# kakaoenterprise/JORLDY

Hardware: AMD Instinct MI355X
Metric: env_steps_per_s (PPO CartPole sync, W=8 workers/GPU, T=128) (higher is better)
Workload: dtype f32

## Files before the change

jorldy_amd/csrc/jh_mlp.hip:

```cpp
#include "jh_ppo_mb.h"
#include "jh_netcore.h"
#include "jh_ppo_finish.h"

typedef float f32x4 __attribute__((ext_vector_type(4)));

namespace {
constexpr int kNormBlocks = 256;
constexpr int kNormSlots = kNormBlocks + 256;
constexpr int kMaxHeadOutputs = 40;
}

constexpr int kL1Rows = 16;
__global__ void __launch_bounds__(256) jh_mlp_l1_kernel(int B, int S, int H, const float* __restrict__ x,
                                                        const int64_t* __restrict__ idx, const float* __restrict__ W1,
                                                        const float* __restrict__ b1, float* __restrict__ h1) {
  __shared__ __attribute__((aligned(16))) float sx[kL1Rows][16];
  const int jb = (H + 255) / 256;
  const int rb = blockIdx.x / jb, j = (blockIdx.x - rb * jb) * 256 + threadIdx.x;
  const int b0 = rb * kL1Rows, nb = b0 + kL1Rows < B ? kL1Rows : B - b0;
  const bool lds_rows = S <= 16;
  if (lds_rows) {
    const int rr = threadIdx.x >> 4, sc = threadIdx.x & 15;
    float v = 0.f;
    if (rr < nb && sc < S) {
// ... 412 lines not shown
__global__ void __launch_bounds__(256) jh_gradnorm_kernel(int64_t n, const float* __restrict__ g,
                                                          float* __restrict__ partial, float* __restrict__ hyper) {
  __shared__ float s_red[16];
  float acc = 0.f;
  const int64_t stride = (int64_t)gridDim.x * 256;
  for (int64_t i0 = (int64_t)blockIdx.x * 256 + threadIdx.x; i0 < n; i0 += 8 * stride) {
    float v[8];
#pragma unroll
    for (int u = 0; u < 8; ++u) {
      const int64_t i = i0 + u * stride;
      v[u] = g[i < n ? i : i0];
    }
#pragma unroll
    for (int u = 0; u < 8; ++u)
      if (i0 + u * stride < n) acc = fmaf(v[u], v[u], acc);
  }
  acc = jh_block_reduce(acc, s_red, JhAdd(), 0.f);
  if (threadIdx.x == 0) partial[blockIdx.x] = acc;
  if (blockIdx.x == 0 && threadIdx.x == 0) jh_adam_advance(hyper);
}

template <bool FUSED>
__global__ void __launch_bounds__(256) jh_adam_kernel(int64_t n, float* __restrict__ p, float* __restrict__ g,
                                                      float* __restrict__ m, float* __restrict__ v,
                                                      const float* __restrict__ partial, int n_partial,
                                                      const float* __restrict__ hyper, float max_norm,
                                                      float* __restrict__ norm_out, const float* __restrict__ part,
                                                      int tiles_m, int64_t n_head) {
  __shared__ float s_red[16];
  const int64_t n4 = n >> 2;
  float4 *p4 = reinterpret_cast<float4*>(p), *g4 = reinterpret_cast<float4*>(g), *m4 = reinterpret_cast<float4*>(m), *v4 = reinterpret_cast<float4*>(v);
  const int64_t i_first = (int64_t)blockIdx.x * 256 + threadIdx.x;
  const int64_t i_fc = i_first < n4 ? i_first : 0;
  const float4 pp0 = p4[i_fc], mm0 = m4[i_fc], vv0 = v4[i_fc], gg0 = g4[i_fc];
  float acc = 0.f;
  bool partials_added = false;
  auto add_partials = [&]() {
    const int ia = threadIdx.x, ib = threadIdx.x + 256;
    const float pa = partial[ia < n_partial ? ia : 0], pb = partial[ib < n_partial ? ib : 0];
    acc += ia < n_partial ? pa : 0.f;
    acc += ib < n_partial ? pb : 0.f;
    for (int i = threadIdx.x + 512; i < n_partial; i += 256) acc += partial[i];
    partials_added = true;
  };
  float4 mine = make_float4(0.f, 0.f, 0.f, 0.f);
  const int64_t h4 = n_head >> 2;
  if (FUSED) {
    const float4* part4 = reinterpret_cast<const float4*>(part);
    constexpr int JU = 3, TU = 16;
    for (int64_t j0 = 0; j0 * 256 < h4; j0 += JU) {
      float4 w[JU][TU];
#pragma unroll
      for (int ju = 0; ju < JU; ++ju) {
        const int64_t i = threadIdx.x + 256 * (j0 + ju);
        const int64_t ic = i < h4 ? i : h4 - 1;
#pragma unroll
        for (int tu = 0; tu < TU; ++tu) w[ju][tu] = part4[(size_t)(tu < tiles_m ? tu : tiles_m - 1) * h4 + ic];
      }
      if (!partials_added) add_partials();
#pragma unroll
      for (int ju = 0; ju < JU; ++ju) {
        const int64_t i = threadIdx.x + 256 * (j0 + ju);
        float4 q = make_float4(0.f, 0.f, 0.f, 0.f);
#pragma unroll
        for (int tu = 0; tu < TU; ++tu)
          if (tu < tiles_m) { q.x += w[ju][tu].x; q.y += w[ju][tu].y; q.z += w[ju][tu].z; q.w += w[ju][tu].w; }
        if (i < h4) {
          acc = fmaf(q.x, q.x, acc); acc = fmaf(q.y, q.y, acc); acc = fmaf(q.z, q.z, acc); acc = fmaf(q.w, q.w, acc);
          if (j0 + ju == blockIdx.x) mine = q;
        }
      }
    }
  }
  if (!partials_added) add_partials();
  const float total = sqrtf(jh_block_reduce(acc, s_red, JhAdd(), 0.f));
  const float bc1 = hyper[5], bc2s = hyper[6];
  float coef = 1.f;
  if (max_norm > 0.f) coef = fminf(max_norm / (total + 1e-6f), 1.f);
  if (blockIdx.x == 0 && threadIdx.x == 0 && norm_out) *norm_out = total;
  const float lr = hyper[JH_HY_LR], b2 = hyper[JH_HY_B2], eps = hyper[JH_HY_EPS];
  const float omb1 = hyper[JH_HY_OMB1], omb2 = hyper[JH_HY_OMB2];
  const float step_size = lr / bc1;
  auto upd = [&](float& pi, float& gi_, float& mi_, float& vi_) {
    const float gi = gi_ * coef;
    gi_ = gi;
    const float mi = mi_ + omb1 * (gi - mi_);
    const float vi = vi_ * b2 + omb2 * gi * gi;
    mi_ = mi;
    vi_ = vi;
    const float denom = sqrtf(vi) / bc2s + eps;
    pi = pi - step_size * (mi / denom);
  };
  for (int64_t i = i_first; i < n4; i += (int64_t)gridDim.x * 256) {
    const bool first = i == i_first;
    float4 pp = first ? pp0 : p4[i], mm = first ? mm0 : m4[i], vv = first ? vv0 : v4[i];
    float4 gg = (FUSED && i < h4) ? mine : (first ? gg0 : g4[i]);
    upd(pp.x, gg.x, mm.x, vv.x); upd(pp.y, gg.y, mm.y, vv.y); upd(pp.z, gg.z, mm.z, vv.z); upd(pp.w, gg.w, mm.w, vv.w);
    p4[i] = pp; g4[i] = gg; m4[i] = mm; v4[i] = vv;
  }
  if (blockIdx.x == 0 && threadIdx.x < (int)(n - (n4 << 2))) {
    const int64_t i = (n4 << 2) + threadIdx.x;
    upd(p[i], g[i], m[i], v[i]);
  }
}

static int64_t pponet_layout(jh_pponet* n) {
  const int64_t S = n->S, H = n->H, A = n->A;
  int64_t o = 0;
  n->o_w1 = o; o += H * S;
  n->o_b1 = o; o += H;
  n->o_w2 = o; o += H * H;
  n->o_b2 = o; o += H;
  n->o_wh0 = o; o += A * H;
  n->o_bh0 = o; o += A;
  if (n->cont) {
    n->o_wh1 = o; o += A * H;
    n->o_bh1 = o; o += A;
  } else {
    n->o_wh1 = n->o_bh1 = -1;
  }
  n->o_wv = o; o += H;
  n->o_bv = o; o += 1;
  return o;
}

JH_EXPORT int64_t jh_pponet_param_count(int32_t S, int32_t H, int32_t A, int32_t continuous) {
// ... 777 lines not shown
```

jorldy_amd/csrc/jh_ppo.hip:

```cpp
#include "jh_common.h"
#include "jh_peer.h"
#include "jh_ppo_finish.h"

__global__ void __launch_bounds__(256) jh_gae_kernel(int W, int T, float gamma, float lambda,
                                                     const float* __restrict__ reward,
                                                     const float* __restrict__ done,
                                                     const float* __restrict__ value,
                                                     const float* __restrict__ next_value,
                                                     float* __restrict__ adv, float* __restrict__ ret,
                                                     int standardize) {
  const int lane = threadIdx.x & 63;
  const int row = blockIdx.x * 4 + (threadIdx.x >> 6);
  if (row >= W) return;
  const size_t base = (size_t)row * (size_t)T;
  const int ntiles = (T + 63) >> 6;
  float carry = 0.f;
  float sum = 0.f;
  for (int k = ntiles - 1; k >= 0; --k) {
    const int t = k * 64 + lane;
    float a = 1.f, b = 0.f, v = 0.f;
    if (t < T) {
      const float r = reward[base + t], d = done[base + t], vn = next_value[base + t];
      v = value[base + t];
      const float nd_g = (1.f - d) * gamma;
// ... 221 lines not shown
  float ratio, surr1, surr2, smin, v, vclip, ret, adv, e1, e2, ent, minp, d_logp_scale;
};

struct NormalD {
  double mu, std, z, th, lp;
};
constexpr int kContCache = 4;
struct DiscRow {
  float m, lse, s;
  NormalD n[kContCache];
};

__device__ __forceinline__ DiscRow disc_prepare(const float* __restrict__ z, int A) {
  DiscRow r;
  float m = z[0];
  for (int k = 1; k < A; ++k) m = fmaxf(m, z[k]);
  float se = 0.f;
  for (int k = 0; k < A; ++k) se += expf(z[k] - m);
  r.m = m;
  r.lse = logf(se);
  float s = 0.f;
  for (int k = 0; k < A; ++k) s += expf((z[k] - m) - r.lse);
  r.s = s;
  return r;
}

__device__ __forceinline__ void disc_terms(const float* __restrict__ z, int k, const DiscRow& r, float& p, float& pn,
                                           float& c, float& lg, bool& inr) {
  p = expf((z[k] - r.m) - r.lse);
  pn = p / r.s;
  inr = (pn >= JH_EPS32) && (pn <= 1.f - JH_EPS32);
  c = fminf(fmaxf(pn, JH_EPS32), 1.f - JH_EPS32);
  lg = logf(c);
}

__global__ void __launch_bounds__(256) jh_logp_discrete_kernel(int64_t M, int A, const float* __restrict__ logits,
                                                               const float* __restrict__ action,
                                                               float* __restrict__ logp) {
  const int64_t i = (int64_t)blockIdx.x * 256 + threadIdx.x;
  if (i >= M) return;
  const float* z = logits + i * A;
  float m = z[0];
  for (int k = 1; k < A; ++k) m = fmaxf(m, z[k]);
  float se = 0.f;
  for (int k = 0; k < A; ++k) se += expf(z[k] - m);
  int a = (int)action[i];
  a = a < 0 ? 0 : (a >= A ? A - 1 : a);
  const float pi = expf((z[a] - m) - logf(se));
  logp[i] = logf(pi);
}

__device__ __forceinline__ NormalD normal_terms(float mu_raw, float ls_raw, float act) {
  NormalD n;
  n.mu = fmin(fmax((double)mu_raw, -5.0), 5.0);
  n.th = tanh((double)ls_raw);
  n.std = exp(n.th);
  const float a = fminf(fmaxf(act, JH_ATANH_LO), JH_ATANH_HI);
  n.z = atanh((double)a);
  const double dm = n.z - n.mu;
  n.lp = -(dm * dm) / (2.0 * n.std * n.std) - log(n.std) - 0.91893853320467274178;
  return n;
}
__device__ __forceinline__ float normal_logp(float mu_raw, float ls_raw, float act, float& mu, float& std, float& z) {
  const NormalD n = normal_terms(mu_raw, ls_raw, act);
  mu = (float)n.mu; std = (float)n.std; z = (float)n.z;
  return (float)n.lp;
// ... 89 lines not shown

struct RowIn {
  int64_t r;
  float adv, ret, vold;
  float action, logp_old;
};
template <bool CONT>
__device__ __forceinline__ RowIn ppo_row_load(const PpoArgs<CONT>& a, int i) {
  RowIn in;
  in.r = a.idx ? a.idx[i] : (int64_t)i;
  in.adv = a.adv[in.r]; in.ret = a.ret[in.r]; in.vold = a.value_old[in.r];
  in.action = 0.f; in.logp_old = 0.f;
  if (!CONT) { in.action = a.action[in.r]; in.logp_old = a.logp_old[in.r]; }
  return in;
}

struct ContPre {
  float z0[kContCache], z1[kContCache], act[kContCache], lpo[kContCache];
};
template <bool CONT>
__device__ __forceinline__ ContPre ppo_cont_prefetch(const PpoArgs<CONT>& a, const float* z0, const float* z1, int64_t r) {
  ContPre c;
#pragma unroll
  for (int k = 0; k < kContCache; ++k) {
    const int kk = k < a.A ? k : a.A - 1;
    c.z0[k] = z0[kk]; c.z1[k] = z1[kk]; c.act[k] = a.action[r * a.A + kk]; c.lpo[k] = a.logp_old[r * a.A + kk];
  }
  return c;
}

template <bool CONT>
__device__ __forceinline__ void ppo_row_fwd(const PpoArgs<CONT>& a, const RowIn& in, const float* z0, const float* z1, float v,
                                            RowCommon& rc, float& ent_row, float& minp_row, DiscRow& dr, int& act_k,
                                            const ContPre* pre = nullptr) {
  const int64_t r = in.r;
  const float adv = in.adv, ret = in.ret, vold = in.vold;
  if (!CONT) {
    const float* z = z0;
    dr = disc_prepare(z, a.A);
    int ak = (int)in.action;
    ak = ak < 0 ? 0 : (ak >= a.A ? a.A - 1 : ak);
    act_k = ak;
    float ent = 0.f, logp = 0.f;
    for (int k = 0; k < a.A; ++k) {
      float p, pn, c, lg;
      bool inr;
      disc_terms(z, k, dr, p, pn, c, lg, inr);
      ent += pn * lg;
      if (k == ak) logp = lg;
    }
    ent_row = -ent;
    rc = row_common(logp - in.logp_old, adv, v, vold, ret, a.eps);
    minp_row = expf(logp);
  } else {
    double lsum = 0.0, ent = 0.0;
    float minp = 3.4e38f;
    auto dim = [&](const NormalD& n, float lpo) {
      lsum += n.lp - (double)lpo;
      ent += 0.5 + 0.91893853320467274178 + n.th;
      minp = fminf(minp, (float)exp(n.lp));
    };
    int k0 = 0;
    if (pre) {
#pragma unroll
      for (int k = 0; k < kContCache; ++k)
        if (k < a.A) { dr.n[k] = normal_terms(pre->z0[k], pre->z1[k], pre->act[k]); dim(dr.n[k], pre->lpo[k]); }
      k0 = kContCache;
    }
    for (int k = k0; k < a.A; ++k) {
      const NormalD n = normal_terms(z0[k], z1[k], a.action[r * a.A + k]);
      if (k < kContCache) dr.n[k] = n;
      dim(n, a.logp_old[r * a.A + k]);
    }
    ent_row = (float)ent;
    rc = row_common((float)lsum, adv, v, vold, ret, a.eps);
    minp_row = minp;
  }
}

template <bool CONT>
__device__ __forceinline__ void ppo_row_bwd(const PpoArgs<CONT>& a, int i, const float* z0, const float* z1,
                                            const RowCommon& rc, const DiscRow& dr, int act_k, float w1, float w2,
                                            const ContPre* pre = nullptr) {
  const float invB = 1.f / (float)a.B;
  const float d_ratio = -invB * (rc.g1 * rc.adv + (rc.in_clip ? rc.g2 * rc.adv : 0.f));
  const float d_logp = d_ratio * rc.ratio;
  if (a.defer_dv2) {
    a.gv[(size_t)i * a.ldv] = a.vf * (2.f * (rc.v - rc.ret) * invB);
    a.defer_dv2[i] = rc.in_v ? a.vf * (2.f * (rc.vclip - rc.ret) * invB) : 0.f;
  } else {
    const float dv = a.vf * (w1 * 2.f * (rc.v - rc.ret) * invB + (rc.in_v ? w2 * 2.f * (rc.vclip - rc.ret) * invB : 0.f));
    a.gv[(size_t)i * a.ldv] = dv;
  }
  if (!CONT) {
    const float* z = z0;
    const float ce = a.ent * invB;
    float T1 = 0.f;
    for (int k = 0; k < a.A; ++k) {
      float p, pn, c, lg;
      bool inr;
      disc_terms(z, k, dr, p, pn, c, lg, inr);
      const float g_lg = (k == act_k ? d_logp : 0.f) + ce * pn;
      const float g_pn = ce * lg + (inr ? g_lg / c : 0.f);
      T1 += g_pn * p;
    }
    float T2 = 0.f;
    const float s = dr.s;
    for (int k = 0; k < a.A; ++k) {
      float p, pn, c, lg;
      bool inr;
      disc_terms(z, k, dr, p, pn, c, lg, inr);
      const float g_lg = (k == act_k ? d_logp : 0.f) + ce * pn;
      const float g_pn = ce * lg + (inr ? g_lg / c : 0.f);
      const float g_p = g_pn / s - T1 / (s * s);
      T2 += g_p * p;
    }
    for (int k = 0; k < a.A; ++k) {
      float p, pn, c, lg;
      bool inr;
      disc_terms(z, k, dr, p, pn, c, lg, inr);
      const float g_lg = (k == act_k ? d_logp : 0.f) + ce * pn;
      const float g_pn = ce * lg + (inr ? g_lg / c : 0.f);
      const float g_p = g_pn / s - T1 / (s * s);
      a.g0[(size_t)i * a.ldg + k] = g_p * p - p * T2;
    }
  } else {
    const int64_t r = a.idx ? a.idx[i] : (int64_t)i;
    const double ce = -(double)a.ent / (double)(a.B * a.A);
    const double dlp = (double)d_logp;
    auto dim = [&](int k, float mr, const NormalD& n) {
      const double var = n.std * n.std, dm = n.z - n.mu;
      const double d_mu = dlp * dm / var;
      const double d_std = dlp * ((dm * dm - var) / (var * n.std)) + ce / n.std;
      a.g0[(size_t)i * a.ldg + k] = (mr >= -5.f && mr <= 5.f) ? (float)d_mu : 0.f;
      a.g1[(size_t)i * a.ldg + k] = (float)(d_std * n.std * (1.0 - n.th * n.th));
    };
    int k0 = 0;
    if (pre) {
#pragma unroll
      for (int k = 0; k < kContCache; ++k)
        if (k < a.A) dim(k, pre->z0[k], dr.n[k]);
      k0 = kContCache;
    }
    for (int k = k0; k < a.A; ++k) {
      const float mr = z0[k], lr = z1[k];
      const NormalD n = k < kContCache ? dr.n[k] : normal_terms(mr, lr, a.action[r * a.A + k]);
      dim(k, mr, n);
    }
  }
}

__device__ __forceinline__ void ppo_block_reduce6(float (&v)[6], float (*red)[6]) {
  const int lane = threadIdx.x & 63, wid = threadIdx.x >> 6, nw = (blockDim.x + 63) >> 6;
#pragma unroll
  for (int o = 32; o > 0; o >>= 1) {
#pragma unroll
    for (int k = 0; k < 4; ++k) v[k] += __shfl_xor(v[k], o, 64);
    v[4] = fmaxf(v[4], __shfl_xor(v[4], o, 64));
    v[5] = fminf(v[5], __shfl_xor(v[5], o, 64));
  }
  if (lane == 0) {
#pragma unroll
    for (int k = 0; k < 6; ++k) red[wid][k] = v[k];
  }
  __syncthreads();
  float r[6] = {0.f, 0.f, 0.f, 0.f, -3.4e38f, 3.4e38f};
  for (int w = 0; w < nw; ++w) {
#pragma unroll
    for (int k = 0; k < 4; ++k) r[k] += red[w][k];
    r[4] = fmaxf(r[4], red[w][4]);
    r[5] = fminf(r[5], red[w][5]);
  }
#pragma unroll
  for (int k = 0; k < 6; ++k) v[k] = r[k];
}

template <bool CONT, int MAXT>
__global__ void __launch_bounds__(MAXT) jh_ppo_fused_kernel(PpoArgs<CONT> a) {
  __shared__ float s_red6[16][6];
  extern __shared__ __attribute__((aligned(16))) float s_z[];
  const int i = threadIdx.x;
  const bool on = i < a.B;
  const float *z0 = nullptr, *z1 = nullptr;
  float vpred = 0.f;
  const RowIn rin = ppo_row_load<CONT>(a, on ? i : 0);
  if (a.hpart) {
    if (on) {
      float z[8] = {0.f, 0.f, 0.f, 0.f, 0.f, 0.f, 0.f, 0.f};
      const bool wide = a.hp_ld == 8;
      if (!wide) {
        constexpr int TU = MAXT <= 256 ? 32 : 16;
        for (int t0 = 0; t0 < a.hp_tiles; t0 += TU) {
          float4 q0[TU];
#pragma unroll
          for (int u = 0; u < TU; ++u) {
            const int t = t0 + u < a.hp_tiles ? t0 + u : a.hp_tiles - 1;
            q0[u] = *reinterpret_cast<const float4*>(a.hpart + ((size_t)t * a.hp_rows + i) * 4);
          }
#pragma unroll
          for (int u = 0; u < TU; ++u)
            if (t0 + u < a.hp_tiles) { z[0] += q0[u].x; z[1] += q0[u].y; z[2] += q0[u].z; z[3] += q0[u].w; }
        }
      } else {
        constexpr int TU = MAXT <= 256 ? 16 : 8;
        for (int t0 = 0; t0 < a.hp_tiles; t0 += TU) {
          float4 q0[TU], q1[TU];
#pragma unroll
          for (int u = 0; u < TU; ++u) {
            const int t = t0 + u < a.hp_tiles ? t0 + u : a.hp_tiles - 1;
            const float4* q = reinterpret_cast<const float4*>(a.hpart + ((size_t)t * a.hp_rows + i) * 8);
            q0[u] = q[0];
            q1[u] = q[1];
          }
#pragma unroll
          for (int u = 0; u < TU; ++u) {
            if (t0 + u < a.hp_tiles) {
              z[0] += q0[u].x; z[1] += q0[u].y; z[2] += q0[u].z; z[3] += q0[u].w;
              z[4] += q1[u].x; z[5] += q1[u].y; z[6] += q1[u].z; z[7] += q1[u].w;
            }
          }
        }
      }
      float4* dst = reinterpret_cast<float4*>(s_z + (size_t)i * 8);
      dst[0] = make_float4(z[0], z[1], z[2], z[3]);
      dst[1] = make_float4(z[4], z[5], z[6], z[7]);
    }
    __syncthreads();
    z0 = s_z + (size_t)i * 8;
    z1 = z0 + a.A;
    if (on) vpred = z0[CONT ? 2 * a.A : a.A];
  } else if (on) {
    z0 = a.h0 + (size_t)i * a.ldh;
    z1 = CONT ? a.h1 + (size_t)i * a.ldh : nullptr;
    vpred = a.value_pred[(size_t)i * a.ldvp];
  }
  RowCommon rc{};
  DiscRow dr{};
  int act_k = 0;
  float ent_row = 0.f, minp = 3.4e38f;
  if (on) ppo_row_fwd<CONT>(a, rin, z0, z1, vpred, rc, ent_row, minp, dr, act_k);
  const float e1 = on ? (rc.v - rc.ret) * (rc.v - rc.ret) : 0.f;
  const float e2 = on ? (rc.vclip - rc.ret) * (rc.vclip - rc.ret) : 0.f;
  float v6[6] = {on ? rc.smin : 0.f, e1, e2, on ? ent_row : 0.f, on ? rc.ratio : -3.4e38f, on ? minp : 3.4e38f};
  ppo_block_reduce6(v6, s_red6);
  float w1, w2;
  ppo_finish_stats(v6[0], v6[1], v6[2], v6[3], v6[4], v6[5], a.B, CONT ? a.B * a.A : a.B, a.vf, a.ent, w1, w2,
                   threadIdx.x == 0 ? a.stats : nullptr);
  if (a.critic_sums && threadIdx.x == 0) { a.critic_sums[0] = v6[1]; a.critic_sums[1] = v6[2]; }
  if (on) ppo_row_bwd<CONT>(a, i, z0, z1, rc, dr, act_k, w1, w2);
  if (a.hyper_advance && threadIdx.x == blockDim.x - 1) jh_adam_advance(a.hyper_advance);
}

template <bool CONT>
__global__ void __launch_bounds__(256) jh_ppo_fwd_kernel(PpoArgs<CONT> a) {
  __shared__ float s_red6[16][6];
  const int i = blockIdx.x * 256 + threadIdx.x;
  const bool on = i < a.B;
  const int ic = on ? i : a.B - 1;
  RowCommon rc{};
  DiscRow dr{};
  int act_k = 0;
  float ent_row = 0.f, minp = 3.4e38f;
  const float* z0 = a.h0 + (size_t)ic * a.ldh;
  const float* z1 = CONT ? a.h1 + (size_t)ic * a.ldh : nullptr;
  const RowIn rin = ppo_row_load<CONT>(a, ic);
  const float vpred = a.value_pred[(size_t)ic * a.ldvp];
  ContPre pre;
  if (CONT) pre = ppo_cont_prefetch<CONT>(a, z0, z1, rin.r);
  ppo_row_fwd<CONT>(a, rin, z0, z1, vpred, rc, ent_row, minp, dr, act_k, CONT ? &pre : nullptr);
  const float e1 = on ? (rc.v - rc.ret) * (rc.v - rc.ret) : 0.f;
  const float e2 = on ? (rc.vclip - rc.ret) * (rc.vclip - rc.ret) : 0.f;
  float v6[6] = {on ? rc.smin : 0.f, e1, e2, on ? ent_row : 0.f, on ? rc.ratio : -3.4e38f, on ? minp : 3.4e38f};
  ppo_block_reduce6(v6, s_red6);
  if (threadIdx.x == 0) {
    float* p = a.partial + (size_t)blockIdx.x * PPO_NPART;
    p[0] = v6[0]; p[1] = v6[1]; p[2] = v6[2]; p[3] = v6[3]; p[4] = v6[4]; p[5] = v6[5];
  }
}

__device__ __forceinline__ void ppo_reduce_partials(const float* __restrict__ partial, int nb, float* s_red, float& t0, float& t1, float& t2, float& t3,
                                                    float& t4, float& t5) {
  t0 = t1 = t2 = t3 = 0.f; t4 = -3.4e38f; t5 = 3.4e38f;
  for (int b = threadIdx.x; b < nb; b += 256) {
    const float* p = partial + (size_t)b * PPO_NPART;
    t0 += p[0]; t1 += p[1]; t2 += p[2]; t3 += p[3];
    t4 = fmaxf(t4, p[4]); t5 = fminf(t5, p[5]);
  }
  t0 = jh_block_reduce(t0, s_red, JhAdd(), 0.f);
  t1 = jh_block_reduce(t1, s_red, JhAdd(), 0.f);
  t2 = jh_block_reduce(t2, s_red, JhAdd(), 0.f);
  t3 = jh_block_reduce(t3, s_red, JhAdd(), 0.f);
  t4 = jh_block_reduce(t4, s_red, JhMax(), -3.4e38f);
  t5 = jh_block_reduce(t5, s_red, JhMin(), 3.4e38f);
}

__global__ void __launch_bounds__(256) jh_ppo_totals_kernel(const float* __restrict__ partial, int nb, float* __restrict__ totals) {
  __shared__ float s_red[16];
  float t0, t1, t2, t3, t4, t5;
  ppo_reduce_partials(partial, nb, s_red, t0, t1, t2, t3, t4, t5);
  if (threadIdx.x == 0) { totals[0] = t0; totals[1] = t1; totals[2] = t2; totals[3] = t3; totals[4] = t4; totals[5] = t5; }
}

template <bool CONT>
__global__ void __launch_bounds__(256) jh_ppo_bwd_kernel(PpoArgs<CONT> a) {
  const int i = blockIdx.x * 256 + threadIdx.x;
  const bool on = i < a.B;
// ... 15 lines not shown
  ppo_finish_stats(t[0], t[1], t[2], t[3], t[4], t[5], a.B, CONT ? a.B * a.A : a.B, a.vf, a.ent, w1, w2,
                   (blockIdx.x == 0 && threadIdx.x == 0) ? a.stats : nullptr);
  if (a.critic_sums && blockIdx.x == 0 && threadIdx.x == 0) { a.critic_sums[0] = t[1]; a.critic_sums[1] = t[2]; }
  RowCommon rc;
  DiscRow dr{};
  int act_k = 0;
  float ent_row, minp;
  ppo_row_fwd<CONT>(a, rin, z0, z1, vpred, rc, ent_row, minp, dr, act_k, CONT ? &pre : nullptr);
  if (on) ppo_row_bwd<CONT>(a, i, z0, z1, rc, dr, act_k, w1, w2, CONT ? &pre : nullptr);
}

template <bool CONT>
__global__ void __launch_bounds__(256) jh_ppo_onepass_kernel(PpoArgs<CONT> a, unsigned* __restrict__ ticket, float* __restrict__ mix) {
  __shared__ float s_red6[16][6];
  __shared__ float s_red[16];
  __shared__ int s_last;
  const int i = blockIdx.x * 256 + threadIdx.x;
  const bool on = i < a.B;
  const int ic = on ? i : a.B - 1;
  RowCommon rc{};
  DiscRow dr{};
  int act_k = 0;
  float ent_row = 0.f, minp = 3.4e38f;
  const float* z0 = a.h0 + (size_t)ic * a.ldh;
  const float* z1 = CONT ? a.h1 + (size_t)ic * a.ldh : nullptr;
  const RowIn rin = ppo_row_load<CONT>(a, ic);
  const float vpred = a.value_pred[(size_t)ic * a.ldvp];
  ContPre pre;
  if (CONT) pre = ppo_cont_prefetch<CONT>(a, z0, z1, rin.r);
  ppo_row_fwd<CONT>(a, rin, z0, z1, vpred, rc, ent_row, minp, dr, act_k, CONT ? &pre : nullptr);
  const float e1 = on ? (rc.v - rc.ret) * (rc.v - rc.ret) : 0.f;
  const float e2 = on ? (rc.vclip - rc.ret) * (rc.vclip - rc.ret) : 0.f;
  float v6[6] = {on ? rc.smin : 0.f, e1, e2, on ? ent_row : 0.f, on ? rc.ratio : -3.4e38f, on ? minp : 3.4e38f};
  ppo_block_reduce6(v6, s_red6);
  if (threadIdx.x < PPO_NPART && threadIdx.x < 6) {
    float mine = v6[0];
#pragma unroll
    for (int k = 1; k < 6; ++k) mine = threadIdx.x == k ? v6[k] : mine;
    __hip_atomic_store(a.partial + (size_t)blockIdx.x * PPO_NPART + threadIdx.x, mine, __ATOMIC_RELAXED, __HIP_MEMORY_SCOPE_AGENT);
  }
  if (on) ppo_row_bwd<CONT>(a, i, z0, z1, rc, dr, act_k, 0.f, 0.f, CONT ? &pre : nullptr);
  if (!ticket) return;
  asm volatile("s_waitcnt vmcnt(0)" ::: "memory");
  __syncthreads();
  if (threadIdx.x == 0) {
    const unsigned old = __hip_atomic_fetch_add(ticket, 1u, __ATOMIC_RELAXED, __HIP_MEMORY_SCOPE_AGENT);
    s_last = old == gridDim.x - 1;
    if (s_last) __hip_atomic_store(ticket, 0u, __ATOMIC_RELAXED, __HIP_MEMORY_SCOPE_AGENT);
  }
  __syncthreads();
  if (!s_last) return;
  float t[6];
  const int nb = (int)gridDim.x;
  if (nb <= 64) {
    const int lane = threadIdx.x & 63;
    const float* p = a.partial + (size_t)(lane < nb ? lane : 0) * PPO_NPART;
    float q[6];
#pragma unroll
    for (int k = 0; k < 6; ++k) q[k] = __hip_atomic_load(p + k, __ATOMIC_RELAXED, __HIP_MEMORY_SCOPE_AGENT);
    const bool mine = lane < nb;
#pragma unroll
    for (int k = 0; k < 4; ++k) t[k] = mine ? 0.f + q[k] : 0.f;
    t[4] = mine ? fmaxf(-3.4e38f, q[4]) : -3.4e38f;
    t[5] = mine ? fminf(3.4e38f, q[5]) : 3.4e38f;
#pragma unroll
    for (int o = 32; o > 0; o >>= 1) {
#pragma unroll
// ... 33 lines not shown
int jh_ppo_loss_onepass(int continuous, int B, int A, const float* d_head0, const float* d_head1, const float* d_value_pred, const int64_t* d_idx,
                        const float* d_action, const float* d_adv, const float* d_ret, const float* d_value_old, const float* d_logp_old, float eps_clip,
                        float vf_coef, float ent_coef, float* d_g0, float* d_g1, float* d_gv, float* d_dv2, float* d_mix, unsigned* d_ticket, float* d_partial,
                        float* d_stats, hipStream_t st) {
  JH_ARG(B > 0 && A > 0 && d_head0 && d_value_pred && d_g0 && d_gv && d_dv2 && d_partial && (d_ticket ? d_mix != nullptr : B <= 64 * 256));
  const int nb = (B + 255) / 256;
  if (continuous) {
    PpoArgs<true> a{};
    a.B = B; a.A = A; a.h0 = d_head0; a.h1 = d_head1; a.value_pred = d_value_pred; a.ldh = A; a.ldvp = 1; a.idx = d_idx;
    a.action = d_action; a.adv = d_adv; a.ret = d_ret; a.value_old = d_value_old; a.logp_old = d_logp_old;
    a.eps = eps_clip; a.vf = vf_coef; a.ent = ent_coef; a.g0 = d_g0; a.g1 = d_g1; a.gv = d_gv; a.ldg = A; a.ldv = 1;
    a.stats = d_stats; a.defer_dv2 = d_dv2; a.partial = d_partial; a.nb = nb;
    JH_LAUNCH(jh_ppo_onepass_kernel<true>, dim3(nb), dim3(256), 0, st, a, d_ticket, d_mix);
  } else {
    PpoArgs<false> a{};
    a.B = B; a.A = A; a.h0 = d_head0; a.h1 = nullptr; a.value_pred = d_value_pred; a.ldh = A; a.ldvp = 1; a.idx = d_idx;
    a.action = d_action; a.adv = d_adv; a.ret = d_ret; a.value_old = d_value_old; a.logp_old = d_logp_old;
    a.eps = eps_clip; a.vf = vf_coef; a.ent = ent_coef; a.g0 = d_g0; a.g1 = nullptr; a.gv = d_gv; a.ldg = A; a.ldv = 1;
    a.stats = d_stats; a.defer_dv2 = d_dv2; a.partial = d_partial; a.nb = nb;
    JH_LAUNCH(jh_ppo_onepass_kernel<false>, dim3(nb), dim3(256), 0, st, a, d_ticket, d_mix);
  }
  JH_LAUNCH_CHECK();
  return JH_OK;
}

template <bool CONT>
static int ppo_launch(jh_ctx* ctx, PpoArgs<CONT>& a, hipStream_t st) {
  if (a.ldh == 0) a.ldh = a.A;
  if (a.ldvp == 0) a.ldvp = 1;
  if (a.B <= 1024) {
    const int threads = ((a.B + 63) / 64) * 64;
    a.nb = 1;
    const size_t lds = a.hpart ? sizeof(float) * 8 * (size_t)a.B : 0;
    if (threads <= 256) JH_LAUNCH((jh_ppo_fused_kernel<CONT, 256>), dim3(1), dim3(threads), lds, st, a);
    else JH_LAUNCH((jh_ppo_fused_kernel<CONT, 1024>), dim3(1), dim3(threads), lds, st, a);
    JH_LAUNCH_CHECK();
    return JH_OK;
  }
  a.nb = (a.B + 255) / 256;
  void* scratch = nullptr;
  int rc = jh_ctx_scratch(ctx, sizeof(float) * (PPO_NPART * (size_t)a.nb + 8), &scratch);
  if (rc) return rc;
  a.partial = (float*)scratch;
  JH_LAUNCH(jh_ppo_fwd_kernel<CONT>, dim3(a.nb), dim3(256), 0, st, a);
  JH_LAUNCH_CHECK();
  if (a.nb > 64) {
    float* totals = a.partial + PPO_NPART * (size_t)a.nb;
    JH_LAUNCH(jh_ppo_totals_kernel, dim3(1), dim3(256), 0, st, a.partial, a.nb, totals);
    JH_LAUNCH_CHECK();
    a.totals = totals;
  }
  JH_LAUNCH(jh_ppo_bwd_kernel<CONT>, dim3(a.nb), dim3(256), 0, st, a);
  JH_LAUNCH_CHECK();
  return JH_OK;
}

JH_EXPORT int jh_ppo_loss_discrete(jh_ctx* ctx, int32_t B, int32_t A, const float* d_logits, const float* d_value_pred,
                                   const int64_t* d_idx, const float* d_action, const float* d_adv, const float* d_ret,
                                   const float* d_value_old, const float* d_logp_old, float eps_clip, float vf_coef,
                                   float ent_coef, float* d_grad_logits, float* d_grad_value, float* d_stats,
                                   jh_stream stream) {
  JH_ARG(ctx && d_logits && d_value_pred && d_action && d_adv && d_ret && d_value_old && d_logp_old);
  JH_ARG(d_grad_logits && d_grad_value);
  JH_ARG(B > 0 && A > 0);
  PpoArgs<false> a{};
  a.B = B; a.A = A; a.h0 = d_logits; a.h1 = nullptr; a.value_pred = d_value_pred; a.idx = d_idx;
  a.action = d_action; a.adv = d_adv; a.ret = d_ret; a.value_old = d_value_old; a.logp_old = d_logp_old;
// ... 201 lines not shown
```

jorldy_amd/csrc/jh_ppo_mb.hip:

```cpp
#include "jh_ppo_mb.h"

typedef float f32x4 __attribute__((ext_vector_type(4)));

struct PmbFwd {
  int M, H, S;
  const float* x;
  const int64_t* x_rows;
  const float *W1, *b1, *W2, *b2;
  const float* h1_in;
  float* h1_out;
  float* h2_out;
  const float* wh[8];
  const float* hb[8];
  int n_out;
  float* part;
  int part_rows, part_ld;
};

template <int SV, bool GEN, int U>
__global__ void __launch_bounds__(256) jh_pmb_fwd_kernel(PmbFwd g) {
  constexpr bool VEC = SV == 1 || SV == 2;
  constexpr int XS = SV == 3 ? 16 : 8;
  __shared__ float s_acc[4][64][4];
  extern __shared__ __attribute__((aligned(16))) float s_dyn[];
// ... 19 lines not shown
  const int wi0 = lane * 4 < n_el ? lane * 4 : 0, wi1 = (lane + 64) * 4 < n_el ? (lane + 64) * 4 : 0;
  const int wi2 = (lane + 128) * 4 < n_el ? (lane + 128) * 4 : 0, wi3 = (lane + 192) * 4 < n_el ? (lane + 192) * 4 : 0;
  const int bi0 = 4 * lane < kn ? 4 * lane : 0;
  if (GEN && VEC) {
    const int kb0 = kn > 0 ? kbeg : 0;
    const float* src = g.W1 + (size_t)kb0 * g.S;
    w1t0 = *reinterpret_cast<const float4*>(src + wi0);
    w1t1 = *reinterpret_cast<const float4*>(src + wi1);
    w1t2 = *reinterpret_cast<const float4*>(src + wi2);
    w1t3 = *reinterpret_cast<const float4*>(src + wi3);
    b1t = *reinterpret_cast<const float4*>(g.b1 + kb0 + bi0);
    __builtin_amdgcn_sched_barrier(0);
  }
  if (GEN) {
    if (VEC) {
#pragma unroll
      for (int q = 0; q < SV; ++q) {
        const float4 v = *reinterpret_cast<const float4*>(g.x + row * g.S + 4 * q);
        xr[4 * q] = v.x; xr[4 * q + 1] = v.y; xr[4 * q + 2] = v.z; xr[4 * q + 3] = v.w;
      }
    } else {
#pragma unroll
      for (int s = 0; s < XS; ++s) xr[s] = s < g.S ? g.x[row * g.S + s] : 0.f;
    }
  }
  float4 bw[U];
#pragma unroll
  for (int u = 0; u < U; ++u) {
    const int kb = kbeg + 16 * u + 4 * kq;
    const int kc = kb < kend ? kb : (kbeg < K ? kbeg : 0);
    bw[u] = *reinterpret_cast<const float4*>(g.W2 + (size_t)n * K + kc);
  }
  const float b2 = g.b2[n];
  float whv[8];
#pragma unroll
  for (int o = 0; o < 8; ++o) whv[o] = o < g.n_out ? g.wh[o][n] : 0.f;
  if (GEN) {
    if (VEC) {
      *reinterpret_cast<float4*>(w1s + wi0) = w1t0;
      *reinterpret_cast<float4*>(w1s + wi1) = w1t1;
      *reinterpret_cast<float4*>(w1s + wi2) = w1t2;
      *reinterpret_cast<float4*>(w1s + wi3) = w1t3;
      for (int i = (lane + 64 * WB) * 4; i < n_el; i += 256) *reinterpret_cast<float4*>(w1s + i) = *reinterpret_cast<const float4*>(g.W1 + (size_t)kbeg * g.S + i);
      *reinterpret_cast<float4*>(b1s + bi0) = b1t;
      for (int i = 4 * (lane + 64); i < kn; i += 256) *reinterpret_cast<float4*>(b1s + i) = *reinterpret_cast<const float4*>(g.b1 + kbeg + i);
    } else {
      const float* src = g.W1 + (size_t)kbeg * g.S;
      if (SV == 3) {
        for (int i = lane; i < n_el; i += 64) {
          const int rr = i / g.S, cc = i - rr * g.S;
          w1s[rr * ws + cc] = src[i];
        }
        for (int i = lane; i < kn * (ws - g.S); i += 64) {
          const int rr = i / (ws - g.S), cc = g.S + (i - rr * (ws - g.S));
          w1s[rr * ws + cc] = 0.f;
        }
      } else {
        for (int i = lane; i < n_el; i += 64) w1s[i] = src[i];
      }
      for (int i = lane; i < kn; i += 64) b1s[i] = g.b1[kbeg + i];
    }
    __builtin_amdgcn_wave_barrier();
    __builtin_amdgcn_fence(__ATOMIC_RELEASE, "workgroup");
  }
  f32x4 acc = (f32x4){0.f, 0.f, 0.f, 0.f};
  const bool st_h1 = GEN && g.h1_out && tn == 0;
  for (int k0 = kbeg; k0 < kend; k0 += 16 * U) {
    float4 av[U], bwn[U];
    if (!GEN) {
// ... 61 lines not shown
    }
    if (more) {
#pragma unroll
      for (int u = 0; u < U; ++u) bw[u] = bwn[u];
    }
  }
#pragma unroll
  for (int i = 0; i < 4; ++i) s_acc[wid][lane][i] = acc[i];
  __syncthreads();
  if (wid != 0) return;
  float hv[4];
#pragma unroll
  for (int i = 0; i < 4; ++i) {
    const int mm = m0 + kq * 4 + i;
    float v = ((s_acc[0][lane][i] + s_acc[1][lane][i]) + s_acc[2][lane][i]) + s_acc[3][lane][i];
    v += b2;
    v = v > 0.f ? v : 0.f;
    hv[i] = mm < g.M ? v : 0.f;
    if (mm < g.M && g.h2_out) g.h2_out[(size_t)mm * K + n] = v;
  }
#pragma unroll
  for (int o = 0; o < 8; ++o) {
    if (o >= g.n_out) break;
    const float w = whv[o];
#pragma unroll
    for (int i = 0; i < 4; ++i) {
      float p = hv[i] * w;
      p += __shfl_xor(p, 1, 64);
      p += __shfl_xor(p, 2, 64);
      p += __shfl_xor(p, 4, 64);
      p += __shfl_xor(p, 8, 64);
      const int mm = m0 + kq * 4 + i;
      if (r == 0 && mm < g.M) {
        if (tn == 0) p += *g.hb[o];
        g.part[((size_t)tn * g.part_rows + mm) * g.part_ld + o] = p;
      }
    }
  }
}

__global__ void __launch_bounds__(256) jh_pmb_heads_finish_kernel(int M, int tiles, int part_rows, int part_ld, const float* __restrict__ part,
                                                                  int A, int cont, float* __restrict__ h0, float* __restrict__ h1,
                                                                  float* __restrict__ v) {
  const int i = blockIdx.x * 256 + threadIdx.x;
  if (i >= M) return;
  float z[8] = {0.f, 0.f, 0.f, 0.f, 0.f, 0.f, 0.f, 0.f};
  const bool wide = part_ld == 8;
  for (int t0 = 0; t0 < tiles; t0 += 8) {
    float4 q0[8], q1[8];
#pragma unroll
    for (int u = 0; u < 8; ++u) {
      const int t = t0 + u < tiles ? t0 + u : tiles - 1;
      const float4* q = reinterpret_cast<const float4*>(part + ((size_t)t * part_rows + i) * part_ld);
      q0[u] = q[0];
      if (wide) q1[u] = q[1];
    }
#pragma unroll
    for (int u = 0; u < 8; ++u) {
      if (t0 + u < tiles) {
        z[0] += q0[u].x; z[1] += q0[u].y; z[2] += q0[u].z; z[3] += q0[u].w;
        if (wide) { z[4] += q1[u].x; z[5] += q1[u].y; z[6] += q1[u].z; z[7] += q1[u].w; }
      }
    }
  }
#pragma unroll
  for (int k = 0; k < 8; ++k) {
    if (k < A) h0[(size_t)i * A + k] = z[k];
// ... 346 lines not shown
  }
  if (!do_norm) return;
  if (blockIdx.x == 0 && threadIdx.x < (int)(n - (n4 << 2))) {
    const float v = grads[(n4 << 2) + threadIdx.x];
    acc = fmaf(v, v, acc);
  }
  acc = jh_block_reduce(acc, s_red, JhAdd(), 0.f);
  if (threadIdx.x == 0) partial[blockIdx.x] = acc;
  if (blockIdx.x == 0 && threadIdx.x == 0) jh_adam_advance(hyper);
}

bool jh_pmb_eligible(const jh_pponet* n, int B) { return n->H % 32 == 0 && B > 0 && B <= n->max_rows && n->n_out <= 8; }

template <int SV, bool GEN>
static int pmb_fwd_launch(const PmbFwd& g, hipStream_t st) {
  const int tiles = ((g.M + 15) / 16) * (g.H / 16);
  const int kper = ((g.H + 63) / 64) * 16;
  const double fl = 2.0 * g.M * (double)g.H * ((GEN ? g.S : 0) + g.H + g.n_out);
  const char* nm = g.M > 1024 ? "jh_pmb_fwd_nograd" : "jh_pmb_fwd";
  const size_t lds = GEN ? sizeof(float) * 4 * (size_t)kper * ((SV == 3 ? ((g.S + 3) & ~3) : g.S) + 1) : 0;
  if (kper > 64) JH_LAUNCH_IDEM(nm, fl, (jh_pmb_fwd_kernel<SV, GEN, 8>), dim3(tiles), dim3(256), lds, st, g);
  else if (kper > 32) JH_LAUNCH_IDEM(nm, fl, (jh_pmb_fwd_kernel<SV, GEN, 4>), dim3(tiles), dim3(256), lds, st, g);
  else JH_LAUNCH_IDEM(nm, fl, (jh_pmb_fwd_kernel<SV, GEN, 2>), dim3(tiles), dim3(256), lds, st, g);
  JH_LAUNCH_CHECK();
  return JH_OK;
}

int jh_pmb_forward(jh_pponet* n, int M, const float* d_x, const int64_t* d_idx, const PmbHeads& hd, const float* h1_in,
                   bool store_act, hipStream_t st) {
  PmbFwd g{};
  g.M = M; g.H = n->H; g.S = n->S; g.x = d_x; g.x_rows = d_idx;
  g.W1 = n->params + n->o_w1; g.b1 = n->params + n->o_b1; g.W2 = n->params + n->o_w2; g.b2 = n->params + n->o_b2;
  g.h1_in = h1_in; g.h1_out = store_act ? n->h1 : nullptr; g.h2_out = store_act ? n->h2 : nullptr;
  for (int o = 0; o < hd.n_out; ++o) { g.wh[o] = hd.w[o]; g.hb[o] = hd.b[o]; }
  g.n_out = hd.n_out; g.part = n->fwd_part; g.part_rows = n->max_rows; g.part_ld = hd.n_out <= 4 ? 4 : 8;
  if (h1_in) return pmb_fwd_launch<0, false>(g, st);
  const bool al = (((uintptr_t)d_x) & 15) == 0 && (((uintptr_t)g.W1) & 15) == 0;
  if (n->S == 4 && al) return pmb_fwd_launch<1, true>(g, st);
  if (n->S == 8 && al) return pmb_fwd_launch<2, true>(g, st);
  if (n->S > 8) return pmb_fwd_launch<3, true>(g, st);
  return pmb_fwd_launch<0, true>(g, st);
}

int jh_pmb_heads_finish(jh_pponet* n, int M, float* d_head0, float* d_head1, float* d_value, hipStream_t st) {
  JH_LAUNCH(jh_pmb_heads_finish_kernel, dim3((M + 255) / 256), dim3(256), 0, st, M, n->H / 16, n->max_rows, (n->cont ? 2 * n->A + 1 : n->A + 1) <= 4 ? 4 : 8, n->fwd_part, n->A,
            n->cont, d_head0, d_head1, d_value);
  JH_LAUNCH_CHECK();
  return JH_OK;
}

int jh_pmb_backward(jh_pponet* n, int B, const float* d_x, const int64_t* d_idx, const PmbHeads& hd, bool emit_ssq, hipStream_t st) {
  PmbBwd g{};
  g.B = B; g.H = n->H; g.S = n->S; g.n_out = hd.n_out; g.x = d_x; g.x_rows = d_idx;
  g.h1 = n->h1; g.h2 = n->h2; g.g_all = n->g_all; g.W2 = n->params + n->o_w2;
  g.dW2 = n->grads + n->o_w2; g.db2 = n->grads + n->o_b2;
  for (int o = 0; o < hd.n_out; ++o) { g.wh[o] = hd.w[o]; g.dwh[o] = hd.dw[o]; g.dbh[o] = hd.db[o]; }
  g.part_w1 = n->part_w1;
  g.ssq_part = emit_ssq ? n->ssq_part : nullptr;
  const int t32 = n->H / 32;
  g.n_dh1 = ((B + 15) / 16) * t32;
  g.n_dw2 = t32 * t32;
  const int grid = g.n_dh1 + g.n_dw2;
  static const int u1 = getenv("JH_PMB_U1") ? atoi(getenv("JH_PMB_U1")) : 8;
  const bool deep = u1 >= 8 && n->H >= 512;
  const double fl = 2.0 * B * (double)n->H * (2.0 * n->H + hd.n_out + n->S + 2.0 * hd.n_out);
  if (hd.n_out <= 4) {
    if (deep) JH_LAUNCH_IDEM("jh_pmb_bwd", fl, (jh_pmb_bwd_kernel<4, 8>), dim3(grid), dim3(256), sizeof(float) * 4 * (size_t)n->H, st, g);
// ... 19 lines not shown
```

Before: 1.153 million.

## Keep small-action PPO logits in registers and hoist hyperparameter/head-bias loads

For discrete action counts up to four, the fused PPO kernel now keeps logits, softmax probabilities and logs in a per-thread register struct instead of staging them through shared memory. This removes one __syncthreads and the LDS round trip. The Adam advance moves to a dedicated extra wavefront so it runs in parallel with the row work. The Adam kernel fetches hyperparameters as vector loads earlier, overlapping them with the partial reduction. The MLP forward kernel preloads head weights and biases unconditionally so they leave the inner loop. These are several micro-optimisations aimed at latency-bound tiny kernels, at the cost of extra register pressure and more code paths.

```diff
diff --git a/jorldy_amd/csrc/jh_mlp.hip b/jorldy_amd/csrc/jh_mlp.hip
--- a/jorldy_amd/csrc/jh_mlp.hip
+++ b/jorldy_amd/csrc/jh_mlp.hip
@@ -468,8 +468,17 @@
   float4 *p4 = reinterpret_cast<float4*>(p), *g4 = reinterpret_cast<float4*>(g), *m4 = reinterpret_cast<float4*>(m), *v4 = reinterpret_cast<float4*>(v);
   const int64_t i_first = (int64_t)blockIdx.x * 256 + threadIdx.x;
   const int64_t i_fc = i_first < n4 ? i_first : 0;
+  const int64_t stride = (int64_t)gridDim.x * 256;
   const float4 pp0 = p4[i_fc], mm0 = m4[i_fc], vv0 = v4[i_fc], gg0 = g4[i_fc];
   float acc = 0.f;
+  float4 hy0 = make_float4(0.f, 0.f, 0.f, 0.f), hy1 = hy0;
+  float hy8 = 0.f;
+  auto fetch_hyper = [&]() {
+    int lane_zero;
+    asm volatile("v_mov_b32 %0, 0" : "=v"(lane_zero));
+    const float4* hy4 = reinterpret_cast<const float4*>(hyper + lane_zero);
+    hy0 = hy4[0]; hy1 = hy4[1]; hy8 = hyper[lane_zero + 8];
+  };
   bool partials_added = false;
   auto add_partials = [&]() {
     const int ia = threadIdx.x, ib = threadIdx.x + 256;
@@ -494,6 +503,7 @@
         for (int tu = 0; tu < TU; ++tu) w[ju][tu] = part4[(size_t)(tu < tiles_m ? tu : tiles_m - 1) * h4 + ic];
       }
       if (!partials_added) add_partials();
+      fetch_hyper();
 #pragma unroll
       for (int ju = 0; ju < JU; ++ju) {
         const int64_t i = threadIdx.x + 256 * (j0 + ju);
@@ -509,13 +519,14 @@
     }
   }
   if (!partials_added) add_partials();
+  if (!FUSED) fetch_hyper();
+  asm volatile("" ::"s"(max_norm), "s"(norm_out), "s"(n), "s"(p), "s"(g), "s"(m), "s"(v), "s"(stride));
   const float total = sqrtf(jh_block_reduce(acc, s_red, JhAdd(), 0.f));
-  const float bc1 = hyper[5], bc2s = hyper[6];
+  const float lr = hy0.x, b2 = hy0.z, eps = hy0.w, bc1 = hy1.y, bc2s = hy1.z;
+  const float omb1 = hy1.w, omb2 = hy8;
   float coef = 1.f;
   if (max_norm > 0.f) coef = fminf(max_norm / (total + 1e-6f), 1.f);
   if (blockIdx.x == 0 && threadIdx.x == 0 && norm_out) *norm_out = total;
-  const float lr = hyper[JH_HY_LR], b2 = hyper[JH_HY_B2], eps = hyper[JH_HY_EPS];
-  const float omb1 = hyper[JH_HY_OMB1], omb2 = hyper[JH_HY_OMB2];
   const float step_size = lr / bc1;
   auto upd = [&](float& pi, float& gi_, float& mi_, float& vi_) {
     const float gi = gi_ * coef;
@@ -527,7 +538,7 @@
     const float denom = sqrtf(vi) / bc2s + eps;
     pi = pi - step_size * (mi / denom);
   };
-  for (int64_t i = i_first; i < n4; i += (int64_t)gridDim.x * 256) {
+  for (int64_t i = i_first; i < n4; i += stride) {
     const bool first = i == i_first;
     float4 pp = first ? pp0 : p4[i], mm = first ? mm0 : m4[i], vv = first ? vv0 : v4[i];
     float4 gg = (FUSED && i < h4) ? mine : (first ? gg0 : g4[i]);
diff --git a/jorldy_amd/csrc/jh_ppo.hip b/jorldy_amd/csrc/jh_ppo.hip
--- a/jorldy_amd/csrc/jh_ppo.hip
+++ b/jorldy_amd/csrc/jh_ppo.hip
@@ -277,6 +277,41 @@
   inr = (pn >= JH_EPS32) && (pn <= 1.f - JH_EPS32);
   c = fminf(fmaxf(pn, JH_EPS32), 1.f - JH_EPS32);
   lg = logf(c);
+}
+
+constexpr int kDiscCache = 4;
+struct DiscReg {
+  float z[kDiscCache];
+  float m, lse, s;
+  float p[kDiscCache], pn[kDiscCache], c[kDiscCache], lg[kDiscCache];
+  bool inr[kDiscCache];
+};
+
+__device__ __forceinline__ void disc_reg_prepare(DiscReg& t, int A) {
+  float m = t.z[0];
+#pragma unroll
+  for (int k = 1; k < kDiscCache; ++k)
+    if (k < A) m = fmaxf(m, t.z[k]);
+  float se = 0.f;
+#pragma unroll
+  for (int k = 0; k < kDiscCache; ++k)
+    if (k < A) se += expf(t.z[k] - m);
+  t.m = m;
+  t.lse = logf(se);
+  float s = 0.f;
+#pragma unroll
+  for (int k = 0; k < kDiscCache; ++k) {
+    t.p[k] = 0.f;
+    if (k < A) { t.p[k] = expf((t.z[k] - m) - t.lse); s += t.p[k]; }
+  }
+  t.s = s;
+#pragma unroll
+  for (int k = 0; k < kDiscCache; ++k) {
+    t.pn[k] = t.p[k] / s;
+    t.inr[k] = (t.pn[k] >= JH_EPS32) && (t.pn[k] <= 1.f - JH_EPS32);
+    t.c[k] = fminf(fmaxf(t.pn[k], JH_EPS32), 1.f - JH_EPS32);
+    t.lg[k] = logf(t.c[k]);
+  }
 }
 
 __global__ void __launch_bounds__(256) jh_logp_discrete_kernel(int64_t M, int A, const float* __restrict__ logits,
@@ -432,10 +467,27 @@
 template <bool CONT>
 __device__ __forceinline__ void ppo_row_fwd(const PpoArgs<CONT>& a, const RowIn& in, const float* z0, const float* z1, float v,
                                             RowCommon& rc, float& ent_row, float& minp_row, DiscRow& dr, int& act_k,
-                                            const ContPre* pre = nullptr) {
+                                            const ContPre* pre = nullptr, DiscReg* dreg = nullptr) {
   const int64_t r = in.r;
   const float adv = in.adv, ret = in.ret, vold = in.vold;
-  if (!CONT) {
+  if (!CONT && dreg) {
+    disc_reg_prepare(*dreg, a.A);
+    dr.m = dreg->m; dr.lse = dreg->lse; dr.s = dreg->s;
+    int ak = (int)in.action;
+    ak = ak < 0 ? 0 : (ak >= a.A ? a.A - 1 : ak);
+    act_k = ak;
+    float ent = 0.f, logp = 0.f;
+#pragma unroll
+    for (int k = 0; k < kDiscCache; ++k) {
+      if (k < a.A) {
+        ent += dreg->pn[k] * dreg->lg[k];
+        if (k == ak) logp = dreg->lg[k];
+      }
+    }
+    ent_row = -ent;
+    rc = row_common(logp - in.logp_old, adv, v, vold, ret, a.eps);
+    minp_row = expf(logp);
+  } else if (!CONT) {
     const float* z = z0;
     dr = disc_prepare(z, a.A);
     int ak = (int)in.action;
@@ -481,7 +533,7 @@
 template <bool CONT>
 __device__ __forceinline__ void ppo_row_bwd(const PpoArgs<CONT>& a, int i, const float* z0, const float* z1,
                                             const RowCommon& rc, const DiscRow& dr, int act_k, float w1, float w2,
-                                            const ContPre* pre = nullptr) {
+                                            const ContPre* pre = nullptr, const DiscReg* dreg = nullptr) {
   const float invB = 1.f / (float)a.B;
   const float d_ratio = -invB * (rc.g1 * rc.adv + (rc.in_clip ? rc.g2 * rc.adv : 0.f));
   const float d_logp = d_ratio * rc.ratio;
@@ -492,7 +544,26 @@
     const float dv = a.vf * (w1 * 2.f * (rc.v - rc.ret) * invB + (rc.in_v ? w2 * 2.f * (rc.vclip - rc.ret) * invB : 0.f));
     a.gv[(size_t)i * a.ldv] = dv;
   }
-  if (!CONT) {
+  if (!CONT && dreg) {
+    const float ce = a.ent * invB;
+    const float s = dr.s;
+    float g_pn[kDiscCache], T1 = 0.f;
+#pragma unroll
+    for (int k = 0; k < kDiscCache; ++k) {
+      const float g_lg = (k == act_k ? d_logp : 0.f) + ce * dreg->pn[k];
+      g_pn[k] = ce * dreg->lg[k] + (dreg->inr[k] ? g_lg / dreg->c[k] : 0.f);
+      if (k < a.A) T1 += g_pn[k] * dreg->p[k];
+    }
+    float g_p[kDiscCache], T2 = 0.f;
+#pragma unroll
+    for (int k = 0; k < kDiscCache; ++k) {
+      g_p[k] = g_pn[k] / s - T1 / (s * s);
+      if (k < a.A) T2 += g_p[k] * dreg->p[k];
+    }
+#pragma unroll
+    for (int k = 0; k < kDiscCache; ++k)
+      if (k < a.A) a.g0[(size_t)i * a.ldg + k] = g_p[k] * dreg->p[k] - dreg->p[k] * T2;
+  } else if (!CONT) {
     const float* z = z0;
     const float ce = a.ent * invB;
     float T1 = 0.f;
@@ -550,8 +621,8 @@
   }
 }
 
-__device__ __forceinline__ void ppo_block_reduce6(float (&v)[6], float (*red)[6]) {
-  const int lane = threadIdx.x & 63, wid = threadIdx.x >> 6, nw = (blockDim.x + 63) >> 6;
+__device__ __forceinline__ void ppo_block_reduce6(float (&v)[6], float (*red)[6], int nw) {
+  const int lane = threadIdx.x & 63, wid = threadIdx.x >> 6;
 #pragma unroll
   for (int o = 32; o > 0; o >>= 1) {
 #pragma unroll
@@ -575,18 +646,31 @@
   for (int k = 0; k < 6; ++k) v[k] = r[k];
 }
 
+constexpr int ppo_fused_threads(int maxt) { return maxt <= 256 ? maxt + 64 : maxt; }
 template <bool CONT, int MAXT>
-__global__ void __launch_bounds__(MAXT) jh_ppo_fused_kernel(PpoArgs<CONT> a) {
+__global__ void __launch_bounds__(ppo_fused_threads(MAXT)) jh_ppo_fused_kernel(PpoArgs<CONT> a) {
   __shared__ float s_red6[16][6];
   extern __shared__ __attribute__((aligned(16))) float s_z[];
   const int i = threadIdx.x;
+  int nw = (blockDim.x + 63) >> 6;
+  if (MAXT <= 256 && a.hyper_advance) {
+    --nw;
+    if (i >= nw * 64) {
+      if (i == nw * 64) jh_adam_advance(a.hyper_advance);
+      return;
+    }
+  }
   const bool on = i < a.B;
+  const bool reg = !CONT && a.A <= kDiscCache;
   const float *z0 = nullptr, *z1 = nullptr;
   float vpred = 0.f;
+  DiscReg dreg;
+#pragma unroll
+  for (int k = 0; k < kDiscCache; ++k) dreg.z[k] = 0.f;
   const RowIn rin = ppo_row_load<CONT>(a, on ? i : 0);
   if (a.hpart) {
+    float z[8] = {0.f, 0.f, 0.f, 0.f, 0.f, 0.f, 0.f, 0.f};
     if (on) {
-      float z[8] = {0.f, 0.f, 0.f, 0.f, 0.f, 0.f, 0.f, 0.f};
       const bool wide = a.hp_ld == 8;
       if (!wide) {
         constexpr int TU = MAXT <= 256 ? 32 : 16;
@@ -621,34 +705,55 @@
           }
         }
       }
-      float4* dst = reinterpret_cast<float4*>(s_z + (size_t)i * 8);
-      dst[0] = make_float4(z[0], z[1], z[2], z[3]);
-      dst[1] = make_float4(z[4], z[5], z[6], z[7]);
-    }
-    __syncthreads();
-    z0 = s_z + (size_t)i * 8;
-    z1 = z0 + a.A;
-    if (on) vpred = z0[CONT ? 2 * a.A : a.A];
+    }
+    if (reg) {
+#pragma unroll
+      for (int k = 0; k < kDiscCache; ++k) dreg.z[k] = z[k];
+#pragma unroll
+      for (int k = 1; k <= kDiscCache; ++k)
+        if (k == a.A) vpred = z[k];
+    } else {
+      if (on) {
+        float4* dst = reinterpret_cast<float4*>(s_z + (size_t)i * 8);
+        dst[0] = make_float4(z[0], z[1], z[2], z[3]);
+        dst[1] = make_float4(z[4], z[5], z[6], z[7]);
+      }
+      __syncthreads();
+      z0 = s_z + (size_t)i * 8;
+      z1 = z0 + a.A;
+      if (on) vpred = z0[CONT ? 2 * a.A : a.A];
+    }
   } else if (on) {
     z0 = a.h0 + (size_t)i * a.ldh;
     z1 = CONT ? a.h1 + (size_t)i * a.ldh : nullptr;
+    if (reg) {
+#pragma unroll
+      for (int k = 0; k < kDiscCache; ++k) dreg.z[k] = z0[k < a.A ? k : a.A - 1];
+    }
     vpred = a.value_pred[(size_t)i * a.ldvp];
   }
   RowCommon rc{};
   DiscRow dr{};
   int act_k = 0;
   float ent_row = 0.f, minp = 3.4e38f;
-  if (on) ppo_row_fwd<CONT>(a, rin, z0, z1, vpred, rc, ent_row, minp, dr, act_k);
+  if (on) {
+    if (reg) ppo_row_fwd<CONT>(a, rin, z0, z1, vpred, rc, ent_row, minp, dr, act_k, nullptr, &dreg);
+    else ppo_row_fwd<CONT>(a, rin, z0, z1, vpred, rc, ent_row, minp, dr, act_k);
+  }
   const float e1 = on ? (rc.v - rc.ret) * (rc.v - rc.ret) : 0.f;
   const float e2 = on ? (rc.vclip - rc.ret) * (rc.vclip - rc.ret) : 0.f;
+  asm volatile("" ::"s"(a.B), "s"(a.A), "s"(a.vf), "s"(a.ent), "s"(a.stats), "s"(a.critic_sums), "s"(a.defer_dv2), "s"(a.g0), "s"(a.g1), "s"(a.gv), "s"(a.ldg), "s"(a.ldv));
   float v6[6] = {on ? rc.smin : 0.f, e1, e2, on ? ent_row : 0.f, on ? rc.ratio : -3.4e38f, on ? minp : 3.4e38f};
-  ppo_block_reduce6(v6, s_red6);
+  ppo_block_reduce6(v6, s_red6, nw);
   float w1, w2;
   ppo_finish_stats(v6[0], v6[1], v6[2], v6[3], v6[4], v6[5], a.B, CONT ? a.B * a.A : a.B, a.vf, a.ent, w1, w2,
                    threadIdx.x == 0 ? a.stats : nullptr);
   if (a.critic_sums && threadIdx.x == 0) { a.critic_sums[0] = v6[1]; a.critic_sums[1] = v6[2]; }
-  if (on) ppo_row_bwd<CONT>(a, i, z0, z1, rc, dr, act_k, w1, w2);
-  if (a.hyper_advance && threadIdx.x == blockDim.x - 1) jh_adam_advance(a.hyper_advance);
+  if (on) {
+    if (reg) ppo_row_bwd<CONT>(a, i, z0, z1, rc, dr, act_k, w1, w2, nullptr, &dreg);
+    else ppo_row_bwd<CONT>(a, i, z0, z1, rc, dr, act_k, w1, w2);
+  }
+  if (MAXT > 256 && a.hyper_advance && threadIdx.x == blockDim.x - 1) jh_adam_advance(a.hyper_advance);
 }
 
 template <bool CONT>
@@ -671,7 +776,7 @@
   const float e1 = on ? (rc.v - rc.ret) * (rc.v - rc.ret) : 0.f;
   const float e2 = on ? (rc.vclip - rc.ret) * (rc.vclip - rc.ret) : 0.f;
   float v6[6] = {on ? rc.smin : 0.f, e1, e2, on ? ent_row : 0.f, on ? rc.ratio : -3.4e38f, on ? minp : 3.4e38f};
-  ppo_block_reduce6(v6, s_red6);
+  ppo_block_reduce6(v6, s_red6, (blockDim.x + 63) >> 6);
   if (threadIdx.x == 0) {
     float* p = a.partial + (size_t)blockIdx.x * PPO_NPART;
     p[0] = v6[0]; p[1] = v6[1]; p[2] = v6[2]; p[3] = v6[3]; p[4] = v6[4]; p[5] = v6[5];
@@ -753,7 +858,7 @@
   const float e1 = on ? (rc.v - rc.ret) * (rc.v - rc.ret) : 0.f;
   const float e2 = on ? (rc.vclip - rc.ret) * (rc.vclip - rc.ret) : 0.f;
   float v6[6] = {on ? rc.smin : 0.f, e1, e2, on ? ent_row : 0.f, on ? rc.ratio : -3.4e38f, on ? minp : 3.4e38f};
-  ppo_block_reduce6(v6, s_red6);
+  ppo_block_reduce6(v6, s_red6, (blockDim.x + 63) >> 6);
   if (threadIdx.x < PPO_NPART && threadIdx.x < 6) {
     float mine = v6[0];
 #pragma unroll
@@ -853,7 +958,7 @@
     const int threads = ((a.B + 63) / 64) * 64;
     a.nb = 1;
     const size_t lds = a.hpart ? sizeof(float) * 8 * (size_t)a.B : 0;
-    if (threads <= 256) JH_LAUNCH((jh_ppo_fused_kernel<CONT, 256>), dim3(1), dim3(threads), lds, st, a);
+    if (threads <= 256) JH_LAUNCH((jh_ppo_fused_kernel<CONT, 256>), dim3(1), dim3(threads + (a.hyper_advance ? 64 : 0)), lds, st, a);
     else JH_LAUNCH((jh_ppo_fused_kernel<CONT, 1024>), dim3(1), dim3(threads), lds, st, a);
     JH_LAUNCH_CHECK();
     return JH_OK;
diff --git a/jorldy_amd/csrc/jh_ppo_mb.hip b/jorldy_amd/csrc/jh_ppo_mb.hip
--- a/jorldy_amd/csrc/jh_ppo_mb.hip
+++ b/jorldy_amd/csrc/jh_ppo_mb.hip
@@ -75,9 +75,15 @@
     bw[u] = *reinterpret_cast<const float4*>(g.W2 + (size_t)n * K + kc);
   }
   const float b2 = g.b2[n];
-  float whv[8];
-#pragma unroll
-  for (int o = 0; o < 8; ++o) whv[o] = o < g.n_out ? g.wh[o][n] : 0.f;
+  float whv[8], hbv[8];
+#pragma unroll
+  for (int o = 0; o < 4; ++o) { whv[o] = g.wh[o][n]; hbv[o] = *g.hb[o]; }
+#pragma unroll
+  for (int o = 4; o < 8; ++o) whv[o] = hbv[o] = 0.f;
+  if (g.part_ld == 8) {
+#pragma unroll
+    for (int o = 4; o < 8; ++o) { whv[o] = g.wh[o][n]; hbv[o] = *g.hb[o]; }
+  }
   if (GEN) {
     if (VEC) {
       *reinterpret_cast<float4*>(w1s + wi0) = w1t0;
@@ -205,7 +211,7 @@
       p += __shfl_xor(p, 8, 64);
       const int mm = m0 + kq * 4 + i;
       if (r == 0 && mm < g.M) {
-        if (tn == 0) p += *g.hb[o];
+        if (tn == 0) p += hbv[o];
         g.part[((size_t)tn * g.part_rows + mm) * g.part_ld + o] = p;
       }
     }
@@ -618,7 +624,7 @@
   g.M = M; g.H = n->H; g.S = n->S; g.x = d_x; g.x_rows = d_idx;
   g.W1 = n->params + n->o_w1; g.b1 = n->params + n->o_b1; g.W2 = n->params + n->o_w2; g.b2 = n->params + n->o_b2;
   g.h1_in = h1_in; g.h1_out = store_act ? n->h1 : nullptr; g.h2_out = store_act ? n->h2 : nullptr;
-  for (int o = 0; o < hd.n_out; ++o) { g.wh[o] = hd.w[o]; g.hb[o] = hd.b[o]; }
+  for (int o = 0; o < 8; ++o) { g.wh[o] = hd.w[o < hd.n_out ? o : 0]; g.hb[o] = hd.b[o < hd.n_out ? o : 0]; }
   g.n_out = hd.n_out; g.part = n->fwd_part; g.part_rows = n->max_rows; g.part_ld = hd.n_out <= 4 ? 4 : 8;
   if (h1_in) return pmb_fwd_launch<0, false>(g, st);
   const bool al = (((uintptr_t)d_x) & 15) == 0 && (((uintptr_t)g.W1) & 15) == 0;
```

After: 1.224 million (median of 6 runs). 1.06x the previous value.
